# MILVLG/mmnas

Measured on AMD Instinct MI355X. Metric: supernet fwd+bwd steps/sec (VQA arch, bs=64), higher is better.
Workload: dtype f32 (bf16x6 split-operand MFMA, fp32 accumulate); 1 GPU; Net_Search supernet WEIGHT step: sample + fwd + BCE(sum) + bwd (+ gradient all-reduce), HSIZE 256, B=64/GPU, 100x2048 regions + 14 tokens, dropout 0.1 (search_vqa.py:279-292; BASELINE configs[2]); global_batch=64, parallelism=dp1, grad_allreduce=none, rccl_ranks=1, rank_id_sum_ok=True, lstm_fallback=False, dp_rows=1, dp_buckets=3, optimizer_in_step=False, gemm_split=6, hip_force_dev_kernarg=1

## Files before the change

include/mmnas_hip.h:

```cpp
#ifndef MMNAS_HIP_H
#define MMNAS_HIP_H

#include <stddef.h>
#include <stdint.h>

#ifdef __cplusplus
extern "C" {
#endif

#define MMNAS_ABI_VERSION 1

enum {
  MMNAS_OK = 0,
  MMNAS_E_SHAPE = -1,
  MMNAS_E_ARG = -2,
  MMNAS_E_LAUNCH = -3
};

enum {
  MMNAS_F_NORM = 1,
  MMNAS_F_RESIDUAL = 2,
  MMNAS_F_MASK = 4,
  MMNAS_F_REL = 8,
  MMNAS_F_SELF = 16,
// ... 190 lines not shown
  uint64_t seed;
  const float* xq;
  const float* xkv;
  const uint8_t* mask;
  const float* rel;
  const float* Wq; const float* Wk; const float* Wv;
  const float* Wm;
  const float* Wr; const float* br;
  const float* ln_a; const float* ln_b;
  float* y;
  void* save;
  void* ws;
  const float* dy;
  float* dxq;
  float* dxkv;
  float* drel;
  float* dWq; float* dWk; float* dWv; float* dWm;
  float* dWr; float* dbr; float* dln_a; float* dln_b;
  int C;
  const float* Wy; const float* by;
  float* dWy; float* dby;
  const int* q_off; const int* k_off;
  int Mq, Mk;
  const int* rel_tile_off;
  int rel_ntiles, reserved2;
} mmnas_att_op;

typedef struct mmnas_plan {
  size_t save_bytes, ws_fwd_bytes, ws_bwd_bytes;
} mmnas_plan;

int mmnas_set_small_ops(int on);
int mmnas_set_small_bwd(int on);
int mmnas_set_small_ffn(int on);
int mmnas_att_op_plan(const mmnas_att_op* op, mmnas_plan* plan);
int mmnas_att_op_fwd(const mmnas_att_op* op, void* stream);
int mmnas_att_op_bwd(const mmnas_att_op* op, void* stream);

typedef struct mmnas_mlp_op {
  int M, nl;
  int dims[4];
  int flags;
  float drop_p, eps;
  uint64_t seed;
  const float* x;
  const float* W[3];
  const float* b[3];
  const float* ln_a; const float* ln_b;
  float* y;
  void* save; void* ws;
  const float* dy;
  float* dx;
  float* dW[3]; float* db[3];
  float* dln_a; float* dln_b;
} mmnas_mlp_op;

int mmnas_mlp_op_plan(const mmnas_mlp_op* op, mmnas_plan* plan);
int mmnas_mlp_op_fwd(const mmnas_mlp_op* op, void* stream);
int mmnas_mlp_op_bwd(const mmnas_mlp_op* op, void* stream);

#define MMNAS_CHAIN_MAX_OPS 128
enum { MMNAS_CHAIN_ATT = 0, MMNAS_CHAIN_MLP = 1 };
typedef struct mmnas_chain_op {
  int kind, on_y;
  mmnas_att_op att;
  mmnas_mlp_op mlp;
// ... 116 lines not shown
```

mmnas_amd/_lib.py:

```python
import ctypes as C
import logging
import os

import torch

_HERE = os.path.dirname(os.path.abspath(__file__))
LIB_PATH = os.environ.get('MMNAS_LIB_PATH') or os.path.join(_HERE, 'lib', 'libmmnas_hip.so')

log = logging.getLogger('mmnas_amd')


def _launch_configuration():
    name = 'HIP_FORCE_DEV_KERNARG'
    if name in os.environ:
        return os.environ[name], 'inherited'
    if torch.cuda.is_initialized():
        log.warning('mmnas_amd was imported after HIP had initialised and %s is not set: kernel arguments go through host-visible '
                    'memory, the ~300 short launches of a step run 20-40 %% slower.  Export %s=1 or import mmnas / mmnas_amd '
                    'before the first CUDA call.', name, name)
        return None, 'unset_after_hip_init'
    os.environ[name] = '1'
    return '1', 'set_by_library'


# ... 94 lines not shown
                ('Wr', _fp * REL_MULTI_MAX), ('br', _fp * REL_MULTI_MAX), ('biasT', _fp * REL_MULTI_MAX),
                ('dbiasT', _fp * REL_MULTI_MAX), ('dWr', _fp * REL_MULTI_MAX), ('dbr', _fp * REL_MULTI_MAX),
                ('off', _fp), ('tile_off', _fp), ('ntiles', C.c_int), ('reserved', C.c_int), ('ws', _fp)]


class ProfStat(C.Structure):
    _fields_ = [('ms', C.c_double), ('flops', C.c_double), ('bytes', C.c_double), ('launches', C.c_long)]


K_NAMES = ['gemm', 'mha_fwd', 'mha_bwd', 'rel_fwd', 'rel_bwd', 'rowops', 'lstm', 'small_ops']


class Segment(C.Structure):
    _fields_ = [('ptr', _fp), ('offset', C.c_uint64), ('n', C.c_uint64)]


_i, _f, _u32, _u64, _sz = C.c_int, C.c_float, C.c_uint32, C.c_uint64, C.c_size_t
SYMBOLS = {
    'mmnas_abi_version': (_i, []),
    'mmnas_last_error': (C.c_char_p, []),
    'mmnas_dropout_mask': (_i, [_fp, _sz, _f, _u64, _u32, _fp]),
    'mmnas_gemm': (_i, [C.POINTER(GemmDesc), _fp]),
    'mmnas_split_planes': (_i, [_fp, _fp, _sz, _fp]),
    'mmnas_gemm_ln': (_i, [C.POINTER(GemmDesc), _fp, _fp, _fp, _f, _fp]),
    'mmnas_set_gemm_ln': (_i, [_i]),
    'mmnas_gemm_pair': (_i, [C.POINTER(GemmDesc), C.POINTER(GemmDesc), _fp]),
    'mmnas_gemm_reload_tuning': (_i, []),
    'mmnas_lstm_supported': (_i, [_i, _i]),
    'mmnas_lstm_fwd': (_i, [_fp] * 9 + [_i, _i, _i, _i, _fp]),
    'mmnas_lstm_bwd': (_i, [_fp] * 7 + [_i, _i, _i, _fp]),
    'mmnas_lstm_seq_supported': (_i, [_i, _i]),
    'mmnas_set_small_ops': (_i, [_i]),
    'mmnas_set_small_bwd': (_i, [_i]),
    'mmnas_set_small_ffn': (_i, [_i]),
    'mmnas_set_chain_overlap': (_i, [_i]),
    'mmnas_lstm_seq_fwd': (_i, [_fp] * 7 + [_i, _i, _i, _fp]),
    'mmnas_lstm_seq_bwd': (_i, [_fp] * 5 + [_i, _i, _i, _fp]),
    'mmnas_lstm_seq_timed_out': (_i, [_fp]),
    'mmnas_layernorm_fwd': (_i, [_fp, _fp, _fp, _fp, _i, _i, _f, _fp]),
    'mmnas_layernorm_bwd': (_i, [_fp, _fp, _fp, _fp, _fp, _fp, _fp, _fp, _fp, _f, _u64, _u32, _i, _i, _f, _fp]),
    'mmnas_layernorm_bwd_ws_floats': (_sz, [_i, _i]),
    'mmnas_colsum': (_i, [_fp, _fp, _i, _i, _i, _fp]),
    'mmnas_eltwise_fwd': (_i, [_i, _fp, _fp, _sz, _fp]),
    'mmnas_eltwise_bwd': (_i, [_i, _fp, _fp, _fp, _sz, _fp]),
    'mmnas_drop_add': (_i, [_fp, _fp, _fp, _sz, _f, _u64, _u32, _fp]),
    'mmnas_glu_fwd': (_i, [_fp, _fp, _i, _i, _i, _f, _u64, _u32, _fp]),
    'mmnas_glu_bwd': (_i, [_fp, _fp, _fp, _i, _i, _i, _f, _u64, _u32, _fp]),
    'mmnas_rel_bias_fwd': (_i, [_fp, _fp, _fp, _fp, _i, _i, _i, _i, _i, _fp]),
    'mmnas_rel_bias_bwd': (_i, [_fp, _fp, _fp, _fp, _fp, _fp, _fp, _i, _i, _i, _i, _i, _i, _fp]),
    'mmnas_row_is_zero': (_i, [_fp, _fp, C.c_long, _i, _fp]),
    'mmnas_glimpse1_supported': (_i, [_i]),
    'mmnas_glimpse1_bwd_ws_floats': (_sz, [C.c_long, _i]),
    'mmnas_glimpse1_fwd': (_i, [_fp, _fp, _fp, _fp, C.c_long, _i, _fp]),
    'mmnas_glimpse1_bwd': (_i, [_fp, _fp, _fp, _fp, _fp, _fp, _fp, C.c_long, _i, _fp]),
    'mmnas_attflat_pool_fwd': (_i, [_fp, _fp, _fp, _fp, _fp, _i, _i, _i, _i, _fp]),
    'mmnas_attflat_pool_bwd': (_i, [_fp, _fp, _fp, _fp, _fp, _fp, _i, _i, _i, _i, _fp]),
    'mmnas_relation_embedding': (_i, [_fp, _fp, _fp, _i, _i, _fp]),
    'mmnas_semantic_embedding': (_i, [_fp, _fp, _fp, _fp, _i, _i, _i, C.c_long, _fp]),
    'mmnas_onehot_rows': (_i, [_fp, _i, _i, C.POINTER(C.c_int), _fp]),
    'mmnas_mixed_sum_ws_floats': (_sz, []),
    'mmnas_mixed_sum_fwd': (_i, [C.POINTER(_fp), _i, _fp, _fp, _sz, _fp]),
    'mmnas_mixed_sum_bwd': (_i, [C.POINTER(_fp), _i, _fp, _fp, _fp, _i, _fp, _fp, _sz, _fp]),
    'mmnas_alpha_full_step': (_i, [_fp, _fp, _fp, _fp, _fp, _i, _i, _f, _f, _f, _f, _i, _fp]),
    'mmnas_alpha_full_step_wd': (_i, [_fp, _fp, _fp, _fp, _fp, _i, _i, _f, _f, _f, _f, _f, _i, _fp]),
    'mmnas_embedding_bwd': (_i, [_fp, _fp, _fp, C.c_long, _i, C.c_long, _fp]),
    'mmnas_node_mix_fwd': (_i, [_fp, _fp, _fp, _i, _fp, _fp, _i, _i, _f, _fp]),
# ... 111 lines not shown
```

mmnas_amd/csrc/small.hip:

```cpp
#include <string.h>
#include "common.h"

namespace mmnas {

int sk_workspace(hipStream_t st, float** ws, size_t* ws_floats, int** cnt, int* ncnt);

typedef unsigned long long u64_;
typedef unsigned u32x4s __attribute__((ext_vector_type(4)));

struct SaSmallK {
  int B, S, H, flags;
  const float* x; const uint8_t* mask;
  const float* Wq; const float* Wk; const float* Wv; const float* Wm;
  const float* ln_a; const float* ln_b;
  float* Q; float* K; float* V; float* att; float* stats; float* z; float* y;
  float* part; int* cnt;
  DropCfg drop_att, drop_out;
  float eps;
};

__device__ __forceinline__ f32x4 mfma16(float a, float b, f32x4 c) {
  return __builtin_amdgcn_mfma_f32_16x16x4f32(a, b, c, 0, 0, 0);
}
#define MFMA16x4(ACC, AF, BF)        \
  ACC = mfma16(AF.x, BF.x, ACC);     \
  ACC = mfma16(AF.y, BF.y, ACC);     \
  ACC = mfma16(AF.z, BF.z, ACC);     \
  ACC = mfma16(AF.w, BF.w, ACC);

__device__ __forceinline__ void st_agent_f(float* ptr, float v) {
  __hip_atomic_store(ptr, v, __ATOMIC_RELAXED, __HIP_MEMORY_SCOPE_AGENT);
}
__device__ __forceinline__ u64_ ld_agent_u64(const u64_* ptr) {
  return __hip_atomic_load(ptr, __ATOMIC_RELAXED, __HIP_MEMORY_SCOPE_AGENT);
}

template <int D>
__global__ void __launch_bounds__(256, 1) sa_small_fwd_kernel(const SaSmallK p) {
  constexpr int LDX = D + 4, LDH = 68;
  constexpr int KC = 128, NCH = D / KC, SPC = KC / 16;
  constexpr int NTM = D / 64;
  __shared__ __attribute__((aligned(16))) float xs[16 * LDX];
  __shared__ __attribute__((aligned(16))) float qs[16 * LDH];
  __shared__ __attribute__((aligned(16))) float ks[16 * LDH];
  __shared__ __attribute__((aligned(16))) float vs[16 * LDH];
  __shared__ __attribute__((aligned(16))) float os[16 * LDH];
  __shared__ float smask[16];
  __shared__ int s_last;
  const int tid = threadIdx.x, lane = tid & 63, w = tid >> 6, l15 = lane & 15, kq = lane >> 4;
  const int h = blockIdx.x, b = blockIdx.y, S = p.S, H = p.H;
  const size_t row0 = (size_t)b * S;

  const float* const wrow[3] = {p.Wq + (size_t)(64 * h + 16 * w + l15) * D + 4 * kq,
                                p.Wk + (size_t)(64 * h + 16 * w + l15) * D + 4 * kq,
                                p.Wv + (size_t)(64 * h + 16 * w + l15) * D + 4 * kq};
  float4 wb[2][3][SPC];
#pragma unroll
  for (int m = 0; m < 3; ++m)
#pragma unroll
    for (int s = 0; s < SPC; ++s) wb[0][m][s] = *reinterpret_cast<const float4*>(wrow[m] + 16 * s);

  {
    constexpr int F4 = D / 4, N = 16 * F4 / 256;
    float4 xv[N];
#pragma unroll
    for (int i = 0; i < N; ++i) {
      const int f = tid + 256 * i, r = f / F4, c4 = f - r * F4;
      const float4 t = *reinterpret_cast<const float4*>(p.x + (row0 + (r < S ? r : 0)) * D + 4 * c4);
      xv[i] = r < S ? t : make_float4(0.f, 0.f, 0.f, 0.f);
    }
#pragma unroll
    for (int i = 0; i < N; ++i) {
      const int f = tid + 256 * i, r = f / F4, c4 = f - r * F4;
      *reinterpret_cast<float4*>(xs + r * LDX + 4 * c4) = xv[i];
    }
    if (tid < 16) smask[tid] = (p.mask && tid < S && p.mask[row0 + tid]) ? 1.f : 0.f;
  }
  __syncthreads();

  f32x4 acc[3];
#pragma unroll
  for (int m = 0; m < 3; ++m) acc[m] = (f32x4){0.f, 0.f, 0.f, 0.f};
#pragma unroll
  for (int c = 0; c < NCH; ++c) {
    if (c + 1 < NCH) {
#pragma unroll
      for (int m = 0; m < 3; ++m)
#pragma unroll
        for (int s = 0; s < SPC; ++s)
          wb[(c + 1) & 1][m][s] = *reinterpret_cast<const float4*>(wrow[m] + KC * (c + 1) + 16 * s);
    }
    __builtin_amdgcn_sched_barrier(0);
#pragma unroll
    for (int s = 0; s < SPC; ++s) {
      const float4 a = *reinterpret_cast<const float4*>(xs + l15 * LDX + KC * c + 16 * s + 4 * kq);
#pragma unroll
      for (int m = 0; m < 3; ++m) { MFMA16x4(acc[m], a, wb[c & 1][m][s]) }
    }
  }
  float4 wm[NTM][4];
#pragma unroll
  for (int t = 0; t < NTM; ++t)
#pragma unroll
    for (int s = 0; s < 4; ++s)
      wm[t][s] = *reinterpret_cast<const float4*>(p.Wm + (size_t)(64 * t + 16 * w + l15) * D + 64 * h + 16 * s + 4 * kq);
  __builtin_amdgcn_sched_barrier(0);
  {
    float* const dst[3] = {qs, ks, vs};
    float* const gdst[3] = {p.Q, p.K, p.V};
#pragma unroll
    for (int m = 0; m < 3; ++m)
#pragma unroll
      for (int r = 0; r < 4; ++r) {
        const int s = 4 * kq + r;
        dst[m][s * LDH + 16 * w + l15] = acc[m][r];
        if (s < S) gdst[m][(row0 + s) * D + 64 * h + 16 * w + l15] = acc[m][r];
      }
  }
  __syncthreads();

  f32x4 sc = (f32x4){0.f, 0.f, 0.f, 0.f};
#pragma unroll
  for (int s = 0; s < 4; ++s) {
    const float4 kf = *reinterpret_cast<const float4*>(ks + l15 * LDH + 16 * s + 4 * kq);
    const float4 qf = *reinterpret_cast<const float4*>(qs + l15 * LDH + 16 * s + 4 * kq);
    MFMA16x4(sc, kf, qf)
  }
  const int qi = l15;
  const size_t bh = (size_t)b * H + h;
  float mx = -INFINITY;
#pragma unroll
  for (int r = 0; r < 4; ++r) {
    const int key = 4 * kq + r;
    float v = sc[r] * 0.125f;
    if (key < S) { if (smask[key] != 0.f) v = -1e9f; } else v = -INFINITY;
    sc[r] = v;
    mx = fmaxf(mx, v);
  }
  mx = fmaxf(mx, __shfl_xor(mx, 16, 64));
  mx = fmaxf(mx, __shfl_xor(mx, 32, 64));
  float sum = 0.f;
#pragma unroll
  for (int r = 0; r < 4; ++r) { sc[r] = __expf(sc[r] - mx); sum += sc[r]; }
  sum += __shfl_xor(sum, 16, 64);
  sum += __shfl_xor(sum, 32, 64);
  const float inv = 1.0f / sum;
  if (w == 0 && kq == 0 && qi < S) {
    p.stats[(bh * S + qi) * 2] = mx;
    p.stats[(bh * S + qi) * 2 + 1] = inv;
  }
#pragma unroll
  for (int r = 0; r < 4; ++r) {
    float a = sc[r] * inv;
    if (p.drop_att.thresh) a *= drop_mult(p.drop_att, (uint32_t)((bh * S + qi) * S + 4 * kq + r));
    sc[r] = a;
  }
  f32x4 o = (f32x4){0.f, 0.f, 0.f, 0.f};
#pragma unroll
  for (int r = 0; r < 4; ++r) o = mfma16(sc[r], vs[(4 * kq + r) * LDH + 16 * w + l15], o);
#pragma unroll
  for (int r = 0; r < 4; ++r) {
    const int s = 4 * kq + r;
    os[s * LDH + 16 * w + l15] = o[r];
    if (s < S) p.att[(row0 + s) * D + 64 * h + 16 * w + l15] = o[r];
  }
  __syncthreads();

  f32x4 pm[NTM];
#pragma unroll
  for (int t = 0; t < NTM; ++t) pm[t] = (f32x4){0.f, 0.f, 0.f, 0.f};
#pragma unroll
  for (int s = 0; s < 4; ++s) {
    const float4 a = *reinterpret_cast<const float4*>(os + l15 * LDH + 16 * s + 4 * kq);
#pragma unroll
    for (int t = 0; t < NTM; ++t) { MFMA16x4(pm[t], a, wm[t][s]) }
  }
  float* const slot = p.part + (bh * 16) * D;
#pragma unroll
  for (int t = 0; t < NTM; ++t)
#pragma unroll
    for (int r = 0; r < 4; ++r) st_agent_f(slot + (4 * kq + r) * D + 64 * t + 16 * w + l15, pm[t][r]);
  asm volatile("s_waitcnt vmcnt(0)" ::: "memory");
  __syncthreads();
  if (tid == 0) s_last = __hip_atomic_fetch_add(p.cnt + b, 1, __ATOMIC_RELAXED, __HIP_MEMORY_SCOPE_AGENT) == H - 1;
  __syncthreads();
  if (!s_last) return;
  if (tid == 0) __hip_atomic_store(p.cnt + b, 0, __ATOMIC_RELAXED, __HIP_MEMORY_SCOPE_AGENT);

  constexpr int HH = D / 64;
  constexpr int NV = D / 256;
  constexpr int RG = D == 256 ? 4 : 2;
  const bool norm = p.flags & MMNAS_F_NORM, resid = p.flags & MMNAS_F_RESIDUAL;
  const __amdgpu_buffer_rsrc_t prsrc =
      __builtin_amdgcn_make_buffer_rsrc((void*)(p.part + (size_t)b * HH * 16 * D), 0, (unsigned)(HH * 16 * D * 4), 0x00020000);
#pragma unroll 1
  for (int g = 0; g < 4 / RG; ++g) {
    u32x4s t[RG][HH][NV];
#pragma unroll
    for (int rr = 0; rr < RG; ++rr) {
      const int s = min(w + 4 * (g * RG + rr), 15);
#pragma unroll
      for (int hh = 0; hh < HH; ++hh)
#pragma unroll
        for (int i = 0; i < NV; ++i)
          t[rr][hh][i] = __builtin_amdgcn_raw_buffer_load_b128(prsrc, (unsigned)(((hh * 16 + s) * D + 4 * (lane + 64 * i)) * 4), 0, 16 );
    }
#pragma unroll
    for (int rr = 0; rr < RG; ++rr) {
      const int s = w + 4 * (g * RG + rr);
      if (s >= S) continue;
      float v[4 * NV];
#pragma unroll
      for (int i = 0; i < 4 * NV; ++i) v[i] = 0.f;
#pragma unroll
      for (int hh = 0; hh < HH; ++hh)
#pragma unroll
        for (int i = 0; i < NV; ++i) {
          v[4 * i] += __uint_as_float(t[rr][hh][i].x); v[4 * i + 1] += __uint_as_float(t[rr][hh][i].y);
          v[4 * i + 2] += __uint_as_float(t[rr][hh][i].z); v[4 * i + 3] += __uint_as_float(t[rr][hh][i].w);
        }
      float sm = 0.f;
#pragma unroll
      for (int i = 0; i < NV; ++i)
#pragma unroll
        for (int e = 0; e < 4; ++e) {
          const int col = 4 * (lane + 64 * i) + e;
          float x = v[4 * i + e];
          if (p.drop_out.thresh) x *= drop_mult(p.drop_out, (uint32_t)(row0 + s) * (uint32_t)D + (uint32_t)col);
          if (resid) x += xs[s * LDX + col];
          v[4 * i + e] = x;
          sm += x;
        }
      float* const yr = p.y + (row0 + s) * D;
      if (!norm) {
#pragma unroll
        for (int i = 0; i < NV; ++i)
          *reinterpret_cast<float4*>(yr + 4 * (lane + 64 * i)) = make_float4(v[4 * i], v[4 * i + 1], v[4 * i + 2], v[4 * i + 3]);
        continue;
      }
      float* const zr = p.z + (row0 + s) * D;
#pragma unroll
      for (int i = 0; i < NV; ++i)
        *reinterpret_cast<float4*>(zr + 4 * (lane + 64 * i)) = make_float4(v[4 * i], v[4 * i + 1], v[4 * i + 2], v[4 * i + 3]);
      const float mean = wave_sum(sm) / (float)D;
      float ss = 0.f;
#pragma unroll
      for (int i = 0; i < 4 * NV; ++i) { v[i] -= mean; ss += v[i] * v[i]; }
      const float sd = sqrtf(wave_sum(ss) / (float)(D - 1));
      const float invs = 1.0f / (sd + p.eps);
#pragma unroll
      for (int i = 0; i < NV; ++i) {
        const int col = 4 * (lane + 64 * i);
        const float4 av = *reinterpret_cast<const float4*>(p.ln_a + col);
        const float4 bv = *reinterpret_cast<const float4*>(p.ln_b + col);
        *reinterpret_cast<float4*>(yr + col) = make_float4(av.x * v[4 * i] * invs + bv.x, av.y * v[4 * i + 1] * invs + bv.y,
                                                           av.z * v[4 * i + 2] * invs + bv.z, av.w * v[4 * i + 3] * invs + bv.w);
      }
    }
  }
}

struct SaSmallBwdK {
// ... 26 lines not shown
  __shared__ __attribute__((aligned(16))) float dqs[16 * LDH], dks[16 * LDH], dvs[16 * LDH];
  __shared__ __attribute__((aligned(16))) float red[2][4][D];
  __shared__ float smask[16], smx[16], sinv[16], sdel[4][16];
  __shared__ int s_last;
  const int tid = threadIdx.x, lane = tid & 63, w = tid >> 6, l15 = lane & 15, kq = lane >> 4;
  const int h = blockIdx.x, b = blockIdx.y, S = p.S, H = p.H;
  const size_t row0 = (size_t)b * S;
  const size_t bh = (size_t)b * H + h;
  const bool norm = p.flags & MMNAS_F_NORM, resid = p.flags & MMNAS_F_RESIDUAL;
  const bool drop_o = p.drop_out.thresh != 0;

  float4 zv[4][NV], gv[4][NV], av[NV];
#pragma unroll
  for (int g = 0; g < 4; ++g) {
    const int s = min(w + 4 * g, S - 1);
#pragma unroll
    for (int i = 0; i < NV; ++i) {
      const int c = 4 * (lane + 64 * i);
      gv[g][i] = *reinterpret_cast<const float4*>(p.dy + (row0 + s) * D + c);
      zv[g][i] = norm ? *reinterpret_cast<const float4*>(p.z + (row0 + s) * D + c) : make_float4(0.f, 0.f, 0.f, 0.f);
    }
  }
#pragma unroll
  for (int i = 0; i < NV; ++i) av[i] = norm ? *reinterpret_cast<const float4*>(p.ln_a + 4 * (lane + 64 * i)) : make_float4(1.f, 1.f, 1.f, 1.f);
  {
    const int r = tid >> 4, c4 = tid & 15;
    const size_t o = (row0 + (r < S ? r : 0)) * D + 64 * h + 4 * c4;
    float4 q4 = *reinterpret_cast<const float4*>(p.Q + o), k4 = *reinterpret_cast<const float4*>(p.K + o),
           v4 = *reinterpret_cast<const float4*>(p.V + o);
    const bool in = r < S;
    q4.x = in ? q4.x : 0.f; q4.y = in ? q4.y : 0.f; q4.z = in ? q4.z : 0.f; q4.w = in ? q4.w : 0.f;
    k4.x = in ? k4.x : 0.f; k4.y = in ? k4.y : 0.f; k4.z = in ? k4.z : 0.f; k4.w = in ? k4.w : 0.f;
    v4.x = in ? v4.x : 0.f; v4.y = in ? v4.y : 0.f; v4.z = in ? v4.z : 0.f; v4.w = in ? v4.w : 0.f;
    *reinterpret_cast<float4*>(qs + r * LDH + 4 * c4) = q4;
    *reinterpret_cast<float4*>(ks + r * LDH + 4 * c4) = k4;
    *reinterpret_cast<float4*>(vs + r * LDH + 4 * c4) = v4;
    if (tid < 16) {
      smask[tid] = (p.mask && tid < S && p.mask[row0 + tid]) ? 1.f : 0.f;
      smx[tid] = tid < S ? p.stats[(bh * S + tid) * 2] : 0.f;
      sinv[tid] = tid < S ? p.stats[(bh * S + tid) * 2 + 1] : 0.f;
    }
  }
  const float* const wmcol = p.Wm + (size_t)(4 * kq) * D + 64 * h + 16 * w + l15;
  float wmf[2][SPC][4];
#pragma unroll
  for (int s = 0; s < SPC; ++s)
#pragma unroll
    for (int j = 0; j < 4; ++j) wmf[0][s][j] = wmcol[(size_t)(16 * s + j) * D];

  float4 acc_a[NV], acc_b[NV];
#pragma unroll
  for (int i = 0; i < NV; ++i) { acc_a[i] = make_float4(0.f, 0.f, 0.f, 0.f); acc_b[i] = acc_a[i]; }
  auto ln_row = [&](const int g, const float4 (&zrow)[NV], const float4 (&grow)[NV]) __attribute__((always_inline)) {
    const int s = w + 4 * g;
    float4 o[NV];
    if (s >= S) {
#pragma unroll
      for (int i = 0; i < NV; ++i) {
        *reinterpret_cast<float4*>(dts + s * LDX + 4 * (lane + 64 * i)) = make_float4(0.f, 0.f, 0.f, 0.f);
        *reinterpret_cast<float4*>(dzs + s * LDX + 4 * (lane + 64 * i)) = make_float4(0.f, 0.f, 0.f, 0.f);
      }
      return;
    }
    if (norm) {
      float4 v[NV];
      float sm = 0.f;
#pragma unroll
      for (int i = 0; i < NV; ++i) { v[i] = zrow[i]; sm += (v[i].x + v[i].y) + (v[i].z + v[i].w); }
      const float mean = wave_sum(sm) / (float)D;
      float ss = 0.f, sg = 0.f, sgc = 0.f;
#pragma unroll
      for (int i = 0; i < NV; ++i) {
        v[i].x -= mean; v[i].y -= mean; v[i].z -= mean; v[i].w -= mean;
        ss += (v[i].x * v[i].x + v[i].y * v[i].y) + (v[i].z * v[i].z + v[i].w * v[i].w);
        const float gx = grow[i].x * av[i].x, gy = grow[i].y * av[i].y, gz = grow[i].z * av[i].z, gw = grow[i].w * av[i].w;
        sg += (gx + gy) + (gz + gw);
        sgc += (gx * v[i].x + gy * v[i].y) + (gz * v[i].z + gw * v[i].w);
      }
      ss = wave_sum(ss); sg = wave_sum(sg); sgc = wave_sum(sgc);
      const float sd = sqrtf(ss / (float)(D - 1));
      const float sden = sd + p.eps;
      const float inv = 1.0f / sden;
      const float mg = sg / (float)D;
      const float k2 = sgc / ((float)(D - 1) * sd * sden * sden);
#pragma unroll
      for (int i = 0; i < NV; ++i) {
        const float4 gg = grow[i];
        o[i].x = (gg.x * av[i].x - mg) * inv - v[i].x * k2;
        o[i].y = (gg.y * av[i].y - mg) * inv - v[i].y * k2;
        o[i].z = (gg.z * av[i].z - mg) * inv - v[i].z * k2;
        o[i].w = (gg.w * av[i].w - mg) * inv - v[i].w * k2;
        acc_a[i].x += gg.x * v[i].x * inv; acc_a[i].y += gg.y * v[i].y * inv;
        acc_a[i].z += gg.z * v[i].z * inv; acc_a[i].w += gg.w * v[i].w * inv;
        acc_b[i].x += gg.x; acc_b[i].y += gg.y; acc_b[i].z += gg.z; acc_b[i].w += gg.w;
      }
    } else {
#pragma unroll
      for (int i = 0; i < NV; ++i) o[i] = grow[i];
    }
#pragma unroll
    for (int i = 0; i < NV; ++i) {
      const int c = 4 * (lane + 64 * i);
      *reinterpret_cast<float4*>(dzs + s * LDX + c) = o[i];
      if (drop_o) {
        const uint32_t base = (uint32_t)(row0 + s) * (uint32_t)D + (uint32_t)c;
        o[i].x *= drop_mult(p.drop_out, base); o[i].y *= drop_mult(p.drop_out, base + 1);
        o[i].z *= drop_mult(p.drop_out, base + 2); o[i].w *= drop_mult(p.drop_out, base + 3);
      }
      *reinterpret_cast<float4*>(dts + s * LDX + c) = o[i];
    }
  };
  ln_row(0, zv[0], gv[0]); ln_row(1, zv[1], gv[1]); ln_row(2, zv[2], gv[2]); ln_row(3, zv[3], gv[3]);
  if (norm && h == 0) {
#pragma unroll
    for (int i = 0; i < NV; ++i) {
      *reinterpret_cast<float4*>(&red[0][w][4 * (lane + 64 * i)]) = acc_a[i];
      *reinterpret_cast<float4*>(&red[1][w][4 * (lane + 64 * i)]) = acc_b[i];
    }
  }
  __syncthreads();
  if (norm && h == 0 && p.lnpart) {
    for (int idx = tid; idx < 2 * (D / 4); idx += 256) {
      const int wh = idx / (D / 4), c = 4 * (idx - wh * (D / 4));
      const float4 r0 = *reinterpret_cast<const float4*>(&red[wh][0][c]), r1 = *reinterpret_cast<const float4*>(&red[wh][1][c]);
      const float4 r2 = *reinterpret_cast<const float4*>(&red[wh][2][c]), r3 = *reinterpret_cast<const float4*>(&red[wh][3][c]);
      *reinterpret_cast<float4*>(p.lnpart + ((size_t)b * 3 + wh) * D + c) =
          make_float4((r0.x + r1.x) + (r2.x + r3.x), (r0.y + r1.y) + (r2.y + r3.y), (r0.z + r1.z) + (r2.z + r3.z), (r0.w + r1.w) + (r2.w + r3.w));
    }
  }
  if (p.dt) {
    const int r = tid >> 4, c4 = tid & 15;
    if (r < S) *reinterpret_cast<float4*>(p.dt + (row0 + r) * D + 64 * h + 4 * c4) = *reinterpret_cast<const float4*>(dts + r * LDX + 64 * h + 4 * c4);
  }

  f32x4 ga = (f32x4){0.f, 0.f, 0.f, 0.f};
#pragma unroll
  for (int c = 0; c < NCH; ++c) {
    if (c + 1 < NCH) {
#pragma unroll
      for (int s = 0; s < SPC; ++s)
#pragma unroll
        for (int j = 0; j < 4; ++j) wmf[(c + 1) & 1][s][j] = wmcol[(size_t)(KC * (c + 1) + 16 * s + j) * D];
    }
    __builtin_amdgcn_sched_barrier(0);
#pragma unroll
    for (int s = 0; s < SPC; ++s) {
      const float4 a = *reinterpret_cast<const float4*>(dts + l15 * LDX + KC * c + 16 * s + 4 * kq);
      ga = mfma16(a.x, wmf[c & 1][s][0], ga);
      ga = mfma16(a.y, wmf[c & 1][s][1], ga);
      ga = mfma16(a.z, wmf[c & 1][s][2], ga);
      ga = mfma16(a.w, wmf[c & 1][s][3], ga);
    }
  }
#pragma unroll
  for (int r = 0; r < 4; ++r) gs[(4 * kq + r) * LDH + 16 * w + l15] = ga[r];

  const float* const wsrc[3] = {p.Wq, p.Wk, p.Wv};
  float4 wf[2][2][4][NTB];
  auto wload = [&](int u, float4 (&dst)[2][4][NTB]) __attribute__((always_inline)) {
    const float* const base = wsrc[u >> 1] + (size_t)(64 * h + 32 * (u & 1) + 4 * kq) * D + 4 * l15;
#pragma unroll
    for (int s2 = 0; s2 < 2; ++s2)
#pragma unroll
      for (int j = 0; j < 4; ++j)
#pragma unroll
        for (int tb = 0; tb < NTB; ++tb)
          dst[s2][j][tb] = *reinterpret_cast<const float4*>(base + (size_t)(16 * s2 + j) * D + 64 * (w + 4 * tb));
  };
  wload(0, wf[0]);
  __syncthreads();

  f32x4 scT = (f32x4){0.f, 0.f, 0.f, 0.f}, scN = scT, dAT = scT, dAN = scT;
#pragma unroll
  for (int s = 0; s < 4; ++s) {
    const float4 kf = *reinterpret_cast<const float4*>(ks + l15 * LDH + 16 * s + 4 * kq);
    const float4 qf = *reinterpret_cast<const float4*>(qs + l15 * LDH + 16 * s + 4 * kq);
    const float4 vf = *reinterpret_cast<const float4*>(vs + l15 * LDH + 16 * s + 4 * kq);
    const float4 gf = *reinterpret_cast<const float4*>(gs + l15 * LDH + 16 * s + 4 * kq);
    MFMA16x4(scT, kf, qf)
    MFMA16x4(scN, qf, kf)
    MFMA16x4(dAT, vf, gf)
    MFMA16x4(dAN, gf, vf)
  }
  float dzT[4], aN[4], dzN[4];
  {
    const float mx = smx[l15], inv = sinv[l15];
    float pr[4], dm[4], dl = 0.f;
#pragma unroll
    for (int r = 0; r < 4; ++r) {
      const int key = 4 * kq + r;
      const bool ok = l15 < S && key < S;
      float v = scT[r] * 0.125f;
      if (smask[key] != 0.f) v = -1e9f;
      pr[r] = ok ? __expf(v - mx) * inv : 0.f;
      dm[r] = drop_mult(p.drop_att, (uint32_t)((bh * S + l15) * S + key));
      dl += dAT[r] * (pr[r] * dm[r]);
    }
    dl += __shfl_xor(dl, 16, 64);
    dl += __shfl_xor(dl, 32, 64);
#pragma unroll
    for (int r = 0; r < 4; ++r) {
      const int key = 4 * kq + r;
      const bool live = l15 < S && key < S && smask[key] == 0.f;
      dzT[r] = live ? pr[r] * (dAT[r] * dm[r] - dl) * 0.125f : 0.f;
    }
    if (kq == 0) sdel[w][l15] = dl;
  }
  __syncthreads();
  {
    const bool masked = smask[l15] != 0.f;
#pragma unroll
    for (int r = 0; r < 4; ++r) {
      const int q = 4 * kq + r;
      const bool ok = l15 < S && q < S;
      float v = scN[r] * 0.125f;
      if (masked) v = -1e9f;
      const float pr = ok ? __expf(v - smx[q]) * sinv[q] : 0.f;
      const float dm = drop_mult(p.drop_att, (uint32_t)((bh * S + q) * S + l15));
      aN[r] = pr * dm;
      dzN[r] = (ok && !masked) ? pr * (dAN[r] * dm - sdel[w][q]) * 0.125f : 0.f;
    }
  }
  f32x4 dq = (f32x4){0.f, 0.f, 0.f, 0.f}, dk = dq, dv = dq;
#pragma unroll
  for (int r = 0; r < 4; ++r) {
    const int o = (4 * kq + r) * LDH + 16 * w + l15;
    dv = mfma16(aN[r], gs[o], dv);
    dq = mfma16(dzT[r], ks[o], dq);
    dk = mfma16(dzN[r], qs[o], dk);
  }
#pragma unroll
  for (int r = 0; r < 4; ++r) {
    const int s = 4 * kq + r, o = s * LDH + 16 * w + l15;
    dqs[o] = dq[r]; dks[o] = dk[r]; dvs[o] = dv[r];
    if (s < S) {
      const size_t go = (row0 + s) * D + 64 * h + 16 * w + l15;
      p.dQ[go] = dq[r]; p.dK[go] = dk[r]; p.dV[go] = dv[r];
    }
  }
  __syncthreads();

  f32x4 px[NTB][4];
#pragma unroll
  for (int tb = 0; tb < NTB; ++tb)
#pragma unroll
    for (int e = 0; e < 4; ++e) px[tb][e] = (f32x4){0.f, 0.f, 0.f, 0.f};
  const float* const asrc[3] = {dqs, dks, dvs};
#pragma unroll
  for (int u = 0; u < 6; ++u) {
    if (u + 1 < 6) wload(u + 1, wf[(u + 1) & 1]);
    __builtin_amdgcn_sched_barrier(0);
#pragma unroll
    for (int s2 = 0; s2 < 2; ++s2) {
      const float4 a = *reinterpret_cast<const float4*>(asrc[u >> 1] + l15 * LDH + 32 * (u & 1) + 16 * s2 + 4 * kq);
      const float aj[4] = {a.x, a.y, a.z, a.w};
#pragma unroll
      for (int j = 0; j < 4; ++j)
#pragma unroll
        for (int tb = 0; tb < NTB; ++tb) {
          const float4 bw = wf[u & 1][s2][j][tb];
          px[tb][0] = mfma16(aj[j], bw.x, px[tb][0]);
          px[tb][1] = mfma16(aj[j], bw.y, px[tb][1]);
          px[tb][2] = mfma16(aj[j], bw.z, px[tb][2]);
          px[tb][3] = mfma16(aj[j], bw.w, px[tb][3]);
        }
    }
  }
  float* const slot = p.part + (bh * 16) * D;
#pragma unroll
  for (int tb = 0; tb < NTB; ++tb)
#pragma unroll
    for (int r = 0; r < 4; ++r) {
      float* const dst = slot + (4 * kq + r) * D + 64 * (w + 4 * tb) + 4 * l15;
      st_agent_f2(dst, px[tb][0][r], px[tb][1][r]);
      st_agent_f2(dst + 2, px[tb][2][r], px[tb][3][r]);
    }
  asm volatile("s_waitcnt vmcnt(0)" ::: "memory");
  __syncthreads();
  if (tid == 0) s_last = __hip_atomic_fetch_add(p.cnt + b, 1, __ATOMIC_RELAXED, __HIP_MEMORY_SCOPE_AGENT) == H - 1;
  __syncthreads();
  if (!s_last) return;
  if (tid == 0) __hip_atomic_store(p.cnt + b, 0, __ATOMIC_RELAXED, __HIP_MEMORY_SCOPE_AGENT);

  constexpr int RG = D == 256 ? 4 : 2;
  const __amdgpu_buffer_rsrc_t prsrc =
      __builtin_amdgcn_make_buffer_rsrc((void*)(p.part + (size_t)b * HH * 16 * D), 0, (unsigned)(HH * 16 * D * 4), 0x00020000);
#pragma unroll 1
  for (int g = 0; g < 4 / RG; ++g) {
    u32x4s t[RG][HH][NV];
#pragma unroll
    for (int rr = 0; rr < RG; ++rr) {
      const int s = min(w + 4 * (g * RG + rr), 15);
#pragma unroll
      for (int hh = 0; hh < HH; ++hh)
#pragma unroll
        for (int i = 0; i < NV; ++i)
          t[rr][hh][i] = __builtin_amdgcn_raw_buffer_load_b128(prsrc, (unsigned)(((hh * 16 + s) * D + 4 * (lane + 64 * i)) * 4), 0, 16 );
    }
#pragma unroll
    for (int rr = 0; rr < RG; ++rr) {
      const int s = w + 4 * (g * RG + rr);
      if (s >= S) continue;
#pragma unroll
      for (int i = 0; i < NV; ++i) {
        float4 v = make_float4(0.f, 0.f, 0.f, 0.f);
#pragma unroll
        for (int hh = 0; hh < HH; ++hh) {
          v.x += __uint_as_float(t[rr][hh][i].x); v.y += __uint_as_float(t[rr][hh][i].y);
          v.z += __uint_as_float(t[rr][hh][i].z); v.w += __uint_as_float(t[rr][hh][i].w);
        }
        if (resid) {
          const float4 zz = *reinterpret_cast<const float4*>(dzs + s * LDX + 4 * (lane + 64 * i));
          v.x += zz.x; v.y += zz.y; v.z += zz.z; v.w += zz.w;
        }
        *reinterpret_cast<float4*>(p.dx + (row0 + s) * D + 4 * (lane + 64 * i)) = v;
      }
    }
  }
}


struct FfnSmallK {
  int B, M, flags;
  const float* x; const float* W1; const float* b1; const float* W2; const float* b2;
  const float* ln_a; const float* ln_b;
  float* h; float* z; float* y;
  float* part; int* cnt;
  DropCfg drop_h, drop_out;
  float eps;
};

template <int D, int HS>
__global__ void __launch_bounds__(256, HS == 256 ? 1 : 2) ffn_small_fwd_kernel(const FfnSmallK p) {
  constexpr int LDX = D + 4, FF = 4 * D, LDHS = HS + 4, NSL = FF / HS;
  constexpr int KC = 64, SPC = KC / 16, NCH1 = D / KC, NCH2 = HS / KC;
  constexpr int NT1 = HS / 64;
  constexpr int NT2 = D / 64;
  __shared__ __attribute__((aligned(16))) float xs[16 * LDX];
  __shared__ __attribute__((aligned(16))) float hs[16 * LDHS];
  __shared__ int s_last;
  const int tid = threadIdx.x, lane = tid & 63, w = tid >> 6, l15 = lane & 15, kq = lane >> 4;
  const int j = blockIdx.x, b = blockIdx.y;
  const size_t row0 = (size_t)b * 16;
  const int S = min(16, p.M - 16 * b);

// ... 159 lines not shown
#pragma unroll
      for (int i = 0; i < 4 * NV; ++i) { v[i] -= mean; ss += v[i] * v[i]; }
      const float sd = sqrtf(wave_sum(ss) / (float)(D - 1));
      const float invs = 1.0f / (sd + p.eps);
#pragma unroll
      for (int i = 0; i < NV; ++i) {
        const int col = 4 * (lane + 64 * i);
        const float4 av = *reinterpret_cast<const float4*>(p.ln_a + col);
        const float4 bv = *reinterpret_cast<const float4*>(p.ln_b + col);
        *reinterpret_cast<float4*>(yr + col) = make_float4(av.x * v[4 * i] * invs + bv.x, av.y * v[4 * i + 1] * invs + bv.y,
                                                           av.z * v[4 * i + 2] * invs + bv.z, av.w * v[4 * i + 3] * invs + bv.w);
      }
    }
  }
}


static int env_on(const char* name, int dflt) {
  const char* e = getenv(name);
  return e && e[0] ? atoi(e) : dflt;
}
static int g_small_ops = -1;
static bool small_ops_on() {
  if (g_small_ops < 0) g_small_ops = env_on("MMNAS_SMALL_OPS", 1) ? 1 : 0;
  return g_small_ops != 0;
}

bool sa_small_applies(const mmnas_att_op* op) {
  if (!small_ops_on() || op->q_off || op->k_off) return false;
  const int fl = op->flags;
  return (fl & MMNAS_F_SELF) && !(fl & MMNAS_F_REL) && op->Sq == op->Sk && op->Sq <= 16 && op->dh == 64 &&
         op->di == op->d && (op->d == 256 || op->d == 512) && op->xq == op->xkv &&
         op->B * op->H <= 256;
}

int sa_small_fwd(const mmnas_att_op* op, float* Q, float* K, float* V, float* att, float* stats, float* z,
                 hipStream_t st) {
  const int fl = op->flags;
  const bool drop = (fl & MMNAS_F_TRAIN) && op->drop_p > 0.f;
  SaSmallK k;
  memset(&k, 0, sizeof(k));
  k.B = op->B; k.S = op->Sq; k.H = op->H; k.flags = fl;
  k.x = op->xq; k.mask = (fl & MMNAS_F_MASK) ? op->mask : nullptr;
  k.Wq = op->Wq; k.Wk = op->Wk; k.Wv = op->Wv; k.Wm = op->Wm; k.ln_a = op->ln_a; k.ln_b = op->ln_b;
  k.Q = Q; k.K = K; k.V = V; k.att = att; k.stats = stats; k.z = z; k.y = op->y;
  k.drop_att = make_drop(drop ? op->drop_p : 0.f, op->seed, 0);
  k.drop_out = make_drop(drop ? op->drop_p : 0.f, op->seed, 1);
  k.eps = op->eps;
  size_t wsf = 0; int ncnt = 0;
  int rc = sk_workspace(st, &k.part, &wsf, &k.cnt, &ncnt);
  if (rc) return rc;
  MMNAS_REQUIRE((size_t)op->B * op->H * 16 * op->d <= wsf && op->B <= ncnt, MMNAS_E_SHAPE,
                "sa_small_fwd: B=%d H=%d d=%d exceeds the hand-off workspace", op->B, op->H, op->d);
  const double M = (double)op->B * op->Sq, d = op->d;
  ProfScope ps(MMNAS_K_SMALL, 2.0 * M * d * d * 4.0 + 4.0 * M * op->Sq * d, 4.0 * (4.0 * d * d + 7.0 * M * d), st, "sa_small_fwd");
  dim3 grid(op->H, op->B), block(256);
  if (op->d == 256) MMNAS_LAUNCH(sa_small_fwd_kernel<256>, grid, block, 0, st, k);
  else MMNAS_LAUNCH(sa_small_fwd_kernel<512>, grid, block, 0, st, k);
  return check_launch("sa_small_fwd");
}

static int g_small_bwd = -1;
static bool small_bwd_on() {
  if (g_small_bwd < 0) g_small_bwd = env_on("MMNAS_SMALL_BWD", 1) ? 1 : 0;
  return g_small_bwd != 0;
}

bool sa_small_bwd_applies(const mmnas_att_op* op) {
  if (!small_bwd_on() || !sa_small_applies(op)) return false;
  if ((op->flags & MMNAS_F_NORM) && (size_t)op->B * 3 * op->d > mmnas_layernorm_bwd_ws_floats(op->B * op->Sq, op->d)) return false;
  return true;
}

int sa_small_bwd(const mmnas_att_op* op, const float* Q, const float* K, const float* V, const float* stats, const float* z,
                 float* dt_out, float* dQ, float* dK, float* dV, float* lnpart, hipStream_t st) {
  const int fl = op->flags;
  const bool drop = (fl & MMNAS_F_TRAIN) && op->drop_p > 0.f;
  SaSmallBwdK k;
  memset(&k, 0, sizeof(k));
  k.B = op->B; k.S = op->Sq; k.H = op->H; k.flags = fl;
  k.dy = op->dy; k.z = z; k.ln_a = op->ln_a; k.mask = (fl & MMNAS_F_MASK) ? op->mask : nullptr;
  k.Wq = op->Wq; k.Wk = op->Wk; k.Wv = op->Wv; k.Wm = op->Wm;
  k.Q = Q; k.K = K; k.V = V; k.stats = stats;
  k.dt = dt_out; k.dQ = dQ; k.dK = dK; k.dV = dV; k.dx = op->dxq; k.lnpart = lnpart;
  k.drop_att = make_drop(drop ? op->drop_p : 0.f, op->seed, 0);
  k.drop_out = make_drop(drop ? op->drop_p : 0.f, op->seed, 1);
  k.eps = op->eps;
  size_t wsf = 0; int ncnt = 0;
  int rc = sk_workspace(st, &k.part, &wsf, &k.cnt, &ncnt);
  if (rc) return rc;
  MMNAS_REQUIRE((size_t)op->B * op->H * 16 * op->d <= wsf && op->B <= ncnt, MMNAS_E_SHAPE,
// ... 17 lines not shown
}

int ffn_small_fwd(const mmnas_mlp_op* op, float* h, float* z, hipStream_t st) {
  const int fl = op->flags;
  const bool drop = (fl & MMNAS_F_TRAIN) && op->drop_p > 0.f;
  FfnSmallK k;
  memset(&k, 0, sizeof(k));
  k.B = (op->M + 15) / 16; k.M = op->M; k.flags = fl;
  k.x = op->x; k.W1 = op->W[0]; k.b1 = op->b[0]; k.W2 = op->W[1]; k.b2 = op->b[1];
  k.ln_a = op->ln_a; k.ln_b = op->ln_b; k.h = h; k.z = z; k.y = op->y;
  k.drop_h = make_drop(drop ? op->drop_p : 0.f, op->seed, 0);
  k.drop_out = make_drop(drop ? op->drop_p : 0.f, op->seed, 1);
  k.eps = op->eps;
  size_t wsf = 0; int ncnt = 0;
  int rc = sk_workspace(st, &k.part, &wsf, &k.cnt, &ncnt);
  if (rc) return rc;
  const int nsl = g_small_ffn == 2 ? 8 : 4;
  MMNAS_REQUIRE((size_t)k.B * nsl * 16 * 256 <= wsf && k.B <= ncnt, MMNAS_E_SHAPE, "ffn_small_fwd: M=%d exceeds the hand-off workspace", op->M);
  const double M = op->M;
  ProfScope ps(MMNAS_K_SMALL, 2.0 * M * 256.0 * 1024.0 * 2.0, 4.0 * (2.0 * 256.0 * 1024.0 + M * (3.0 * 256.0 + 1024.0)), st, "ffn_small_fwd");
  if (nsl == 8) MMNAS_LAUNCH((ffn_small_fwd_kernel<256, 128>), dim3(8, k.B), dim3(256), 0, st, k);
  else MMNAS_LAUNCH((ffn_small_fwd_kernel<256, 256>), dim3(4, k.B), dim3(256), 0, st, k);
  return check_launch("ffn_small_fwd");
}

}

extern "C" int mmnas_set_small_ffn(int on) {
  const int prev = mmnas::small_ffn_on() ? 1 : 0;
  mmnas::g_small_ffn = on < 0 ? 0 : (on > 2 ? 2 : on);
  return prev;
}

extern "C" int mmnas_set_small_bwd(int on) {
  const int prev = mmnas::small_bwd_on() ? 1 : 0;
  mmnas::g_small_bwd = on ? 1 : 0;
  return prev;
}

extern "C" int mmnas_set_small_ops(int on) {
  const int prev = mmnas::small_ops_on() ? 1 : 0;
  mmnas::g_small_ops = on ? 1 : 0;
  return prev;
}
```

Before: 231.0 steps/s.

## Add opt-in bf16x6 split MFMA path and LDS swizzle to small self-attention

Adds a B16 template variant of the small self-attention forward kernel. It pre-splits x into three bf16 planes in shared memory and computes the QKV and output projections with 16x16x32 bf16 MFMAs (six-product split) instead of the fp32 16x16x4 MFMA. This variant is selected only when MMNAS_SMALL_B16 is set. All shared-memory tiles in the forward and backward kernels now use an XOR column swizzle, which is meant to reduce LDS bank conflicts. The swizzle applies by default and adds index arithmetic; the bf16 path trades extra split work and LDS space for higher MFMA throughput.

```diff
diff --git a/include/mmnas_hip.h b/include/mmnas_hip.h
--- a/include/mmnas_hip.h
+++ b/include/mmnas_hip.h
@@ -246,6 +246,7 @@
 
 int mmnas_set_small_ops(int on);
 int mmnas_set_small_bwd(int on);
+int mmnas_set_small_b16(int on);
 int mmnas_set_small_ffn(int on);
 int mmnas_att_op_plan(const mmnas_att_op* op, mmnas_plan* plan);
 int mmnas_att_op_fwd(const mmnas_att_op* op, void* stream);
diff --git a/mmnas_amd/_lib.py b/mmnas_amd/_lib.py
--- a/mmnas_amd/_lib.py
+++ b/mmnas_amd/_lib.py
@@ -150,6 +150,7 @@
     'mmnas_lstm_seq_supported': (_i, [_i, _i]),
     'mmnas_set_small_ops': (_i, [_i]),
     'mmnas_set_small_bwd': (_i, [_i]),
+    'mmnas_set_small_b16': (_i, [_i]),
     'mmnas_set_small_ffn': (_i, [_i]),
     'mmnas_set_chain_overlap': (_i, [_i]),
     'mmnas_lstm_seq_fwd': (_i, [_fp] * 7 + [_i, _i, _i, _fp]),
diff --git a/mmnas_amd/csrc/small.hip b/mmnas_amd/csrc/small.hip
--- a/mmnas_amd/csrc/small.hip
+++ b/mmnas_amd/csrc/small.hip
@@ -1,5 +1,6 @@
 #include <string.h>
 #include "common.h"
+#include "gemm_split.h"
 
 namespace mmnas {
 
@@ -28,6 +29,26 @@
   ACC = mfma16(AF.z, BF.z, ACC);     \
   ACC = mfma16(AF.w, BF.w, ACC);
 
+__device__ __forceinline__ int swp(int row) { return ((row >> 2) ^ (row >> 3)) & 1; }
+__device__ __forceinline__ int sw4(int row, int col) { return col ^ (swp(row) << 2); }
+
+__device__ __forceinline__ void split8(const float4 a, const float4 b, bf16x8 (&o)[3]) {
+  unsigned w[4][3];
+  split_pair<3>(a.x, a.y, w[0][0], w[0][1], w[0][2]);
+  split_pair<3>(a.z, a.w, w[1][0], w[1][1], w[1][2]);
+  split_pair<3>(b.x, b.y, w[2][0], w[2][1], w[2][2]);
+  split_pair<3>(b.z, b.w, w[3][0], w[3][1], w[3][2]);
+#pragma unroll
+  for (int c = 0; c < 3; ++c) o[c] = __builtin_bit_cast(bf16x8, (u32x4){w[0][c], w[1][c], w[2][c], w[3][c]});
+}
+__device__ __forceinline__ f32x4 mfma6_16(const bf16x8 (&a)[3], const bf16x8 (&b)[3], f32x4 acc) {
+#pragma unroll
+  for (int o = 2; o >= 0; --o)
+#pragma unroll
+    for (int c = 0; c <= o; ++c) acc = __builtin_amdgcn_mfma_f32_16x16x32_bf16(a[c], b[o - c], acc, 0, 0, 0);
+  return acc;
+}
+
 __device__ __forceinline__ void st_agent_f(float* ptr, float v) {
   __hip_atomic_store(ptr, v, __ATOMIC_RELAXED, __HIP_MEMORY_SCOPE_AGENT);
 }
@@ -35,12 +56,14 @@
   return __hip_atomic_load(ptr, __ATOMIC_RELAXED, __HIP_MEMORY_SCOPE_AGENT);
 }
 
-template <int D>
+template <int D, bool B16>
 __global__ void __launch_bounds__(256, 1) sa_small_fwd_kernel(const SaSmallK p) {
   constexpr int LDX = D + 4, LDH = 68;
+  constexpr int RSB = 2 * D + 16, PLB = 16 * RSB;
   constexpr int KC = 128, NCH = D / KC, SPC = KC / 16;
   constexpr int NTM = D / 64;
   __shared__ __attribute__((aligned(16))) float xs[16 * LDX];
+  __shared__ __attribute__((aligned(16))) unsigned char xb[B16 ? 3 * PLB : 16];
   __shared__ __attribute__((aligned(16))) float qs[16 * LDH];
   __shared__ __attribute__((aligned(16))) float ks[16 * LDH];
   __shared__ __attribute__((aligned(16))) float vs[16 * LDH];
@@ -72,7 +95,16 @@
 #pragma unroll
     for (int i = 0; i < N; ++i) {
       const int f = tid + 256 * i, r = f / F4, c4 = f - r * F4;
-      *reinterpret_cast<float4*>(xs + r * LDX + 4 * c4) = xv[i];
+      *reinterpret_cast<float4*>(xs + r * LDX + sw4(r, 4 * c4)) = xv[i];
+      if constexpr (B16) {
+        unsigned a0, a1, a2, b0, b1, b2;
+        split_pair<3>(xv[i].x, xv[i].y, a0, a1, a2);
+        split_pair<3>(xv[i].z, xv[i].w, b0, b1, b2);
+        unsigned char* const d = xb + r * RSB + (((4 * (c4 >> 3) + (c4 & 3)) ^ swp(r)) * 16) + ((c4 >> 2) & 1) * 8;
+        *reinterpret_cast<uint2*>(d) = make_uint2(a0, b0);
+        *reinterpret_cast<uint2*>(d + PLB) = make_uint2(a1, b1);
+        *reinterpret_cast<uint2*>(d + 2 * PLB) = make_uint2(a2, b2);
+      }
     }
     if (tid < 16) smask[tid] = (p.mask && tid < S && p.mask[row0 + tid]) ? 1.f : 0.f;
   }
@@ -91,11 +123,27 @@
           wb[(c + 1) & 1][m][s] = *reinterpret_cast<const float4*>(wrow[m] + KC * (c + 1) + 16 * s);
     }
     __builtin_amdgcn_sched_barrier(0);
-#pragma unroll
-    for (int s = 0; s < SPC; ++s) {
-      const float4 a = *reinterpret_cast<const float4*>(xs + l15 * LDX + KC * c + 16 * s + 4 * kq);
-#pragma unroll
-      for (int m = 0; m < 3; ++m) { MFMA16x4(acc[m], a, wb[c & 1][m][s]) }
+    if constexpr (B16) {
+#pragma unroll
+      for (int j = 0; j < SPC / 2; ++j) {
+        bf16x8 af[3];
+        const unsigned char* const src = xb + l15 * RSB + (((4 * ((KC / 32) * c + j) + kq) ^ swp(l15)) * 16);
+#pragma unroll
+        for (int e = 0; e < 3; ++e) af[e] = *reinterpret_cast<const bf16x8*>(src + e * PLB);
+#pragma unroll
+        for (int m = 0; m < 3; ++m) {
+          bf16x8 bw[3];
+          split8(wb[c & 1][m][2 * j], wb[c & 1][m][2 * j + 1], bw);
+          acc[m] = mfma6_16(af, bw, acc[m]);
+        }
+      }
+    } else {
+#pragma unroll
+      for (int s = 0; s < SPC; ++s) {
+        const float4 a = *reinterpret_cast<const float4*>(xs + l15 * LDX + sw4(l15, KC * c + 16 * s + 4 * kq));
+#pragma unroll
+        for (int m = 0; m < 3; ++m) { MFMA16x4(acc[m], a, wb[c & 1][m][s]) }
+      }
     }
   }
   float4 wm[NTM][4];
@@ -113,7 +161,7 @@
 #pragma unroll
       for (int r = 0; r < 4; ++r) {
         const int s = 4 * kq + r;
-        dst[m][s * LDH + 16 * w + l15] = acc[m][r];
+        dst[m][s * LDH + sw4(s, 16 * w + l15)] = acc[m][r];
         if (s < S) gdst[m][(row0 + s) * D + 64 * h + 16 * w + l15] = acc[m][r];
       }
   }
@@ -122,8 +170,8 @@
   f32x4 sc = (f32x4){0.f, 0.f, 0.f, 0.f};
 #pragma unroll
   for (int s = 0; s < 4; ++s) {
-    const float4 kf = *reinterpret_cast<const float4*>(ks + l15 * LDH + 16 * s + 4 * kq);
-    const float4 qf = *reinterpret_cast<const float4*>(qs + l15 * LDH + 16 * s + 4 * kq);
+    const float4 kf = *reinterpret_cast<const float4*>(ks + l15 * LDH + sw4(l15, 16 * s + 4 * kq));
+    const float4 qf = *reinterpret_cast<const float4*>(qs + l15 * LDH + sw4(l15, 16 * s + 4 * kq));
     MFMA16x4(sc, kf, qf)
   }
   const int qi = l15;
@@ -157,11 +205,11 @@
   }
   f32x4 o = (f32x4){0.f, 0.f, 0.f, 0.f};
 #pragma unroll
-  for (int r = 0; r < 4; ++r) o = mfma16(sc[r], vs[(4 * kq + r) * LDH + 16 * w + l15], o);
+  for (int r = 0; r < 4; ++r) o = mfma16(sc[r], vs[(4 * kq + r) * LDH + sw4(4 * kq + r, 16 * w + l15)], o);
 #pragma unroll
   for (int r = 0; r < 4; ++r) {
     const int s = 4 * kq + r;
-    os[s * LDH + 16 * w + l15] = o[r];
+    os[s * LDH + sw4(s, 16 * w + l15)] = o[r];
     if (s < S) p.att[(row0 + s) * D + 64 * h + 16 * w + l15] = o[r];
   }
   __syncthreads();
@@ -169,11 +217,26 @@
   f32x4 pm[NTM];
 #pragma unroll
   for (int t = 0; t < NTM; ++t) pm[t] = (f32x4){0.f, 0.f, 0.f, 0.f};
-#pragma unroll
-  for (int s = 0; s < 4; ++s) {
-    const float4 a = *reinterpret_cast<const float4*>(os + l15 * LDH + 16 * s + 4 * kq);
-#pragma unroll
-    for (int t = 0; t < NTM; ++t) { MFMA16x4(pm[t], a, wm[t][s]) }
+  if constexpr (B16) {
+#pragma unroll
+    for (int j = 0; j < 2; ++j) {
+      bf16x8 af[3];
+      split8(*reinterpret_cast<const float4*>(os + l15 * LDH + sw4(l15, 32 * j + 4 * kq)),
+             *reinterpret_cast<const float4*>(os + l15 * LDH + sw4(l15, 32 * j + 16 + 4 * kq)), af);
+#pragma unroll
+      for (int t = 0; t < NTM; ++t) {
+        bf16x8 bw[3];
+        split8(wm[t][2 * j], wm[t][2 * j + 1], bw);
+        pm[t] = mfma6_16(af, bw, pm[t]);
+      }
+    }
+  } else {
+#pragma unroll
+    for (int s = 0; s < 4; ++s) {
+      const float4 a = *reinterpret_cast<const float4*>(os + l15 * LDH + sw4(l15, 16 * s + 4 * kq));
+#pragma unroll
+      for (int t = 0; t < NTM; ++t) { MFMA16x4(pm[t], a, wm[t][s]) }
+    }
   }
   float* const slot = p.part + (bh * 16) * D;
 #pragma unroll
@@ -227,7 +290,7 @@
           const int col = 4 * (lane + 64 * i) + e;
           float x = v[4 * i + e];
           if (p.drop_out.thresh) x *= drop_mult(p.drop_out, (uint32_t)(row0 + s) * (uint32_t)D + (uint32_t)col);
-          if (resid) x += xs[s * LDX + col];
+          if (resid) x += xs[s * LDX + sw4(s, col)];
           v[4 * i + e] = x;
           sm += x;
         }
@@ -320,9 +383,9 @@
     q4.x = in ? q4.x : 0.f; q4.y = in ? q4.y : 0.f; q4.z = in ? q4.z : 0.f; q4.w = in ? q4.w : 0.f;
     k4.x = in ? k4.x : 0.f; k4.y = in ? k4.y : 0.f; k4.z = in ? k4.z : 0.f; k4.w = in ? k4.w : 0.f;
     v4.x = in ? v4.x : 0.f; v4.y = in ? v4.y : 0.f; v4.z = in ? v4.z : 0.f; v4.w = in ? v4.w : 0.f;
-    *reinterpret_cast<float4*>(qs + r * LDH + 4 * c4) = q4;
-    *reinterpret_cast<float4*>(ks + r * LDH + 4 * c4) = k4;
-    *reinterpret_cast<float4*>(vs + r * LDH + 4 * c4) = v4;
+    *reinterpret_cast<float4*>(qs + r * LDH + sw4(r, 4 * c4)) = q4;
+    *reinterpret_cast<float4*>(ks + r * LDH + sw4(r, 4 * c4)) = k4;
+    *reinterpret_cast<float4*>(vs + r * LDH + sw4(r, 4 * c4)) = v4;
     if (tid < 16) {
       smask[tid] = (p.mask && tid < S && p.mask[row0 + tid]) ? 1.f : 0.f;
       smx[tid] = tid < S ? p.stats[(bh * S + tid) * 2] : 0.f;
@@ -389,13 +452,13 @@
 #pragma unroll
     for (int i = 0; i < NV; ++i) {
       const int c = 4 * (lane + 64 * i);
-      *reinterpret_cast<float4*>(dzs + s * LDX + c) = o[i];
+      *reinterpret_cast<float4*>(dzs + s * LDX + sw4(s, c)) = o[i];
       if (drop_o) {
         const uint32_t base = (uint32_t)(row0 + s) * (uint32_t)D + (uint32_t)c;
         o[i].x *= drop_mult(p.drop_out, base); o[i].y *= drop_mult(p.drop_out, base + 1);
         o[i].z *= drop_mult(p.drop_out, base + 2); o[i].w *= drop_mult(p.drop_out, base + 3);
       }
-      *reinterpret_cast<float4*>(dts + s * LDX + c) = o[i];
+      *reinterpret_cast<float4*>(dts + s * LDX + sw4(s, c)) = o[i];
     }
   };
   ln_row(0, zv[0], gv[0]); ln_row(1, zv[1], gv[1]); ln_row(2, zv[2], gv[2]); ln_row(3, zv[3], gv[3]);
@@ -418,7 +481,7 @@
   }
   if (p.dt) {
     const int r = tid >> 4, c4 = tid & 15;
-    if (r < S) *reinterpret_cast<float4*>(p.dt + (row0 + r) * D + 64 * h + 4 * c4) = *reinterpret_cast<const float4*>(dts + r * LDX + 64 * h + 4 * c4);
+    if (r < S) *reinterpret_cast<float4*>(p.dt + (row0 + r) * D + 64 * h + 4 * c4) = *reinterpret_cast<const float4*>(dts + r * LDX + sw4(r, 64 * h + 4 * c4));
   }
 
   f32x4 ga = (f32x4){0.f, 0.f, 0.f, 0.f};
@@ -433,7 +496,7 @@
     __builtin_amdgcn_sched_barrier(0);
 #pragma unroll
     for (int s = 0; s < SPC; ++s) {
-      const float4 a = *reinterpret_cast<const float4*>(dts + l15 * LDX + KC * c + 16 * s + 4 * kq);
+      const float4 a = *reinterpret_cast<const float4*>(dts + l15 * LDX + sw4(l15, KC * c + 16 * s + 4 * kq));
       ga = mfma16(a.x, wmf[c & 1][s][0], ga);
       ga = mfma16(a.y, wmf[c & 1][s][1], ga);
       ga = mfma16(a.z, wmf[c & 1][s][2], ga);
@@ -441,7 +504,7 @@
     }
   }
 #pragma unroll
-  for (int r = 0; r < 4; ++r) gs[(4 * kq + r) * LDH + 16 * w + l15] = ga[r];
+  for (int r = 0; r < 4; ++r) gs[(4 * kq + r) * LDH + sw4(4 * kq + r, 16 * w + l15)] = ga[r];
 
   const float* const wsrc[3] = {p.Wq, p.Wk, p.Wv};
   float4 wf[2][2][4][NTB];
@@ -461,10 +524,11 @@
   f32x4 scT = (f32x4){0.f, 0.f, 0.f, 0.f}, scN = scT, dAT = scT, dAN = scT;
 #pragma unroll
   for (int s = 0; s < 4; ++s) {
-    const float4 kf = *reinterpret_cast<const float4*>(ks + l15 * LDH + 16 * s + 4 * kq);
-    const float4 qf = *reinterpret_cast<const float4*>(qs + l15 * LDH + 16 * s + 4 * kq);
-    const float4 vf = *reinterpret_cast<const float4*>(vs + l15 * LDH + 16 * s + 4 * kq);
-    const float4 gf = *reinterpret_cast<const float4*>(gs + l15 * LDH + 16 * s + 4 * kq);
+    const int fo = l15 * LDH + sw4(l15, 16 * s + 4 * kq);
+    const float4 kf = *reinterpret_cast<const float4*>(ks + fo);
+    const float4 qf = *reinterpret_cast<const float4*>(qs + fo);
+    const float4 vf = *reinterpret_cast<const float4*>(vs + fo);
+    const float4 gf = *reinterpret_cast<const float4*>(gs + fo);
     MFMA16x4(scT, kf, qf)
     MFMA16x4(scN, qf, kf)
     MFMA16x4(dAT, vf, gf)
@@ -512,14 +576,14 @@
   f32x4 dq = (f32x4){0.f, 0.f, 0.f, 0.f}, dk = dq, dv = dq;
 #pragma unroll
   for (int r = 0; r < 4; ++r) {
-    const int o = (4 * kq + r) * LDH + 16 * w + l15;
+    const int o = (4 * kq + r) * LDH + sw4(4 * kq + r, 16 * w + l15);
     dv = mfma16(aN[r], gs[o], dv);
     dq = mfma16(dzT[r], ks[o], dq);
     dk = mfma16(dzN[r], qs[o], dk);
   }
 #pragma unroll
   for (int r = 0; r < 4; ++r) {
-    const int s = 4 * kq + r, o = s * LDH + 16 * w + l15;
+    const int s = 4 * kq + r, o = s * LDH + sw4(s, 16 * w + l15);
     dqs[o] = dq[r]; dks[o] = dk[r]; dvs[o] = dv[r];
     if (s < S) {
       const size_t go = (row0 + s) * D + 64 * h + 16 * w + l15;
@@ -540,7 +604,7 @@
     __builtin_amdgcn_sched_barrier(0);
 #pragma unroll
     for (int s2 = 0; s2 < 2; ++s2) {
-      const float4 a = *reinterpret_cast<const float4*>(asrc[u >> 1] + l15 * LDH + 32 * (u & 1) + 16 * s2 + 4 * kq);
+      const float4 a = *reinterpret_cast<const float4*>(asrc[u >> 1] + l15 * LDH + sw4(l15, 32 * (u & 1) + 16 * s2 + 4 * kq));
       const float aj[4] = {a.x, a.y, a.z, a.w};
 #pragma unroll
       for (int j = 0; j < 4; ++j)
@@ -598,7 +662,7 @@
           v.z += __uint_as_float(t[rr][hh][i].z); v.w += __uint_as_float(t[rr][hh][i].w);
         }
         if (resid) {
-          const float4 zz = *reinterpret_cast<const float4*>(dzs + s * LDX + 4 * (lane + 64 * i));
+          const float4 zz = *reinterpret_cast<const float4*>(dzs + s * LDX + sw4(s, 4 * (lane + 64 * i)));
           v.x += zz.x; v.y += zz.y; v.z += zz.z; v.w += zz.w;
         }
         *reinterpret_cast<float4*>(p.dx + (row0 + s) * D + 4 * (lane + 64 * i)) = v;
@@ -824,6 +888,12 @@
   return (fl & MMNAS_F_SELF) && !(fl & MMNAS_F_REL) && op->Sq == op->Sk && op->Sq <= 16 && op->dh == 64 &&
          op->di == op->d && (op->d == 256 || op->d == 512) && op->xq == op->xkv &&
          op->B * op->H <= 256;
+}
+
+static int g_small_b16 = -1;
+static bool small_b16_on() {
+  if (g_small_b16 < 0) g_small_b16 = env_on("MMNAS_SMALL_B16", 0) ? 1 : 0;
+  return g_small_b16 != 0;
 }
 
 int sa_small_fwd(const mmnas_att_op* op, float* Q, float* K, float* V, float* att, float* stats, float* z,
@@ -847,8 +917,13 @@
   const double M = (double)op->B * op->Sq, d = op->d;
   ProfScope ps(MMNAS_K_SMALL, 2.0 * M * d * d * 4.0 + 4.0 * M * op->Sq * d, 4.0 * (4.0 * d * d + 7.0 * M * d), st, "sa_small_fwd");
   dim3 grid(op->H, op->B), block(256);
-  if (op->d == 256) MMNAS_LAUNCH(sa_small_fwd_kernel<256>, grid, block, 0, st, k);
-  else MMNAS_LAUNCH(sa_small_fwd_kernel<512>, grid, block, 0, st, k);
+  if (small_b16_on()) {
+    if (op->d == 256) MMNAS_LAUNCH((sa_small_fwd_kernel<256, true>), grid, block, 0, st, k);
+    else MMNAS_LAUNCH((sa_small_fwd_kernel<512, true>), grid, block, 0, st, k);
+  } else {
+    if (op->d == 256) MMNAS_LAUNCH((sa_small_fwd_kernel<256, false>), grid, block, 0, st, k);
+    else MMNAS_LAUNCH((sa_small_fwd_kernel<512, false>), grid, block, 0, st, k);
+  }
   return check_launch("sa_small_fwd");
 }
 
@@ -932,6 +1007,12 @@
   return prev;
 }
 
+extern "C" int mmnas_set_small_b16(int on) {
+  const int prev = mmnas::small_b16_on() ? 1 : 0;
+  mmnas::g_small_b16 = on ? 1 : 0;
+  return prev;
+}
+
 extern "C" int mmnas_set_small_bwd(int on) {
   const int prev = mmnas::small_bwd_on() ? 1 : 0;
   mmnas::g_small_bwd = on ? 1 : 0;
```

Measured after the change: 230.7 steps/s. No clear change (-0.1%).
